# openai/blocksparse

Hardware: NVIDIA H100
Metric: effective TFLOP/s (2*nnz_blocks*bs^2*N, fprop+bprop+updat) (higher is better)
Workload: dtype bf16

## Files before the change

blocksparse_b200/csrc/tc_xprop2.cuh:

```cuda
#pragma once
#include "tc.cuh"

namespace bsmm {

template <int TB, int MI> struct Xp2Shape {
  static constexpr uint32_t XBYTES = MI * 64 * 32 * 2;
  static constexpr uint32_t WBYTES = 32 * 32 * 2;
  static constexpr uint32_t STAGE = (XBYTES + TB * WBYTES + 1023) / 1024 * 1024;
  static constexpr size_t SMEM = XP_STAGES * STAGE + SMEM_ALIGN_SLACK;
};
constexpr int XP2_REC = 8;

struct Xprop2Params {
  const int32_t* tile_off;
  const int32_t* ent;
  int n_out;
  int w_absent;
  void* y;
  long long y_pitch;
  int N;
};

template <int TB, int MI, bool BF16, bool AXIS0, bool BPROP>
__global__ void __launch_bounds__(XP_THREADS)
tc_xprop2_kernel(const Xprop2Params p, const __grid_constant__ XpropTmaps maps) {
  using Sh = Xp2Shape<TB, MI>;
  constexpr int ST = XP_STAGES, NW = TB * 32;
  extern __shared__ uint8_t smem_raw[];
  __shared__ uint64_t full[ST];
  const uint32_t base = aligned_smem_base(smem_raw);
  const int tid = threadIdx.x, warp = tid / 32, lane = tid % 32;
  const int nt = blockIdx.x, t = blockIdx.y;
  const int first = p.tile_off[t], count = p.tile_off[t + 1] - first;
  const int32_t* ent = p.ent + (size_t)first * XP2_REC;

  auto issue = [&](int e) {
    const int32_t* r = ent + e * XP2_REC;
    const uint32_t st = base + (uint32_t)(e % ST) * Sh::STAGE;
    uint64_t* bar = &full[e % ST];
    ptx::mbar_expect_tx(bar, Sh::XBYTES + TB * Sh::WBYTES);
    if (!AXIS0) {
      ptx::tma_load_2d(st, &maps.x, bar, r[0] * 32, nt * MI * 64);
    } else {
#pragma unroll
      for (int m = 0; m < MI; ++m) ptx::tma_load_2d(st + m * 4096, &maps.x, bar, nt * MI * 64 + m * 64, r[0] * 32);
    }
#pragma unroll
    for (int j = 0; j < TB; ++j) {
      const int wb = r[1 + j];
      ptx::tma_load_2d(st + Sh::XBYTES + j * Sh::WBYTES, &maps.w, bar, 0, (wb < 0 ? p.w_absent : wb) * 32);
    }
  };

  if (tid == 0) {
    for (int i = 0; i < ST; ++i) ptx::mbar_init(&full[i], 1);
    ptx::fence_mbar_init();
    ptx::prefetch_tensormap(&maps.x); ptx::prefetch_tensormap(&maps.w);
  }
  __syncthreads();
  if (tid == 0)
    for (int e = 0; e < count && e < ST; ++e) issue(e);

  float acc[MI][NW / 2];
#pragma unroll
  for (int m = 0; m < MI; ++m)
#pragma unroll
    for (int i = 0; i < NW / 2; ++i) acc[m][i] = 0.f;

  for (int e = 0; e < count; ++e) {
    const uint32_t st = base + (uint32_t)(e % ST) * Sh::STAGE;
    if (!ptx::mbar_wait(&full[e % ST], (uint32_t)(e / ST) & 1)) g_tc_error = 41;
    ptx::wg_fence();
#pragma unroll
    for (int ks = 0; ks < 2; ++ks) {
      const uint64_t bdesc = BPROP ? ptx::make_desc(st + Sh::XBYTES + ks * 32, 16, 512, ptx::SWZ_64B)
                                   : ptx::make_desc(st + Sh::XBYTES + ks * 1024, Sh::WBYTES, 512, ptx::SWZ_64B);
#pragma unroll
      for (int m = 0; m < MI; ++m) {
        const uint64_t adesc = AXIS0 ? ptx::make_desc(st + m * 4096 + ks * 2048, 4096, 1024, ptx::SWZ_128B)
                                     : ptx::make_desc(st + m * 64 * 64 + ks * 32, 16, 512, ptx::SWZ_64B);
        ptx::wgmma<BF16, AXIS0 ? 1 : 0, BPROP ? 0 : 1, NW>(acc[m], adesc, bdesc);
      }
    }
    ptx::wg_commit();
    ptx::wg_wait<1>();
    __syncthreads();
    if (tid == 0 && e >= 1 && e - 1 + ST < count) issue(e - 1 + ST);
  }
  ptx::wg_wait<0>();
#pragma unroll
  for (int m = 0; m < MI; ++m) ptx::wg_fence_regs(acc[m]);

  uint16_t* y = reinterpret_cast<uint16_t*>(p.y);
#pragma unroll
  for (int m = 0; m < MI; ++m)
#pragma unroll
    for (int h = 0; h < 2; ++h) {
      const long long n = (long long)nt * MI * 64 + m * 64 + warp * 16 + lane / 4 + 8 * h;
      if (n >= p.N) continue;
#pragma unroll
      for (int j = 0; j < NW / 8; ++j) {
        const int cl = 8 * j + 2 * (lane % 4);
        const int o = t * TB + cl / 32;
        if (o >= p.n_out) continue;
        const int col = o * 32 + cl % 32;
        const float a = acc[m][4 * j + 2 * h], b = acc[m][4 * j + 2 * h + 1];
        if (!AXIS0) {
          *reinterpret_cast<uint32_t*>(y + n * p.y_pitch + col) = pack2<BF16>(a, b);
        } else {
          y[(long long)col * p.y_pitch + n] = pack1<BF16>(a);
          y[(long long)(col + 1) * p.y_pitch + n] = pack1<BF16>(b);
        }
      }
    }
}

template <int TB, int MI, bool BF16, bool AXIS0, bool BPROP>
int launch_tc_xprop2(const Xprop2Params& p, const XpropTmaps& maps, int n_tiles, cudaStream_t s) {
  auto kern = tc_xprop2_kernel<TB, MI, BF16, AXIS0, BPROP>;
  constexpr size_t smem = Xp2Shape<TB, MI>::SMEM;
  static thread_local uint64_t configured = 0;
  if (int e = ensure_dyn_smem(kern, smem, configured)) return e;
  kern<<<dim3((unsigned)((p.N + MI * 64 - 1) / (MI * 64)), (unsigned)n_tiles), XP_THREADS, smem, s>>>(p, maps);
  return check_launch("wgmma_xprop2_bs32");
}

template <int TB, int MI, bool BF16>
int dispatch_tc_xprop2(const Xprop2Params& p, const XpropTmaps& maps, int n_tiles, bool axis0, bool bprop, cudaStream_t s) {
  if (axis0) return bprop ? launch_tc_xprop2<TB, MI, BF16, true, true>(p, maps, n_tiles, s) : launch_tc_xprop2<TB, MI, BF16, true, false>(p, maps, n_tiles, s);
  return bprop ? launch_tc_xprop2<TB, MI, BF16, false, true>(p, maps, n_tiles, s) : launch_tc_xprop2<TB, MI, BF16, false, false>(p, maps, n_tiles, s);
}

inline int tc_xprop2(int dtype, int axis, int bprop, int n_out, int n_in, int blocks, const void* x, const void* w, void* y,
                     int N, const int32_t* sched, int n_tiles, int variant, int ent_off, cudaStream_t s) {
  if (dtype != BSMM_F16 && dtype != BSMM_BF16) return fail(BSMM_E_ARG, "bsmm_xprop: the wide-tile schedule needs a 16-bit dtype");
  if (variant < 1 || variant > 3) return fail(BSMM_E_ARG, "bsmm_xprop: wide-tile variant %d (1..3)", variant);
  const int tb = variant == 3 ? 4 : 2;
  if (sched == nullptr || n_tiles <= 0 || (long long)n_tiles * tb < n_out || ent_off < n_tiles + 3)
    return fail(BSMM_E_ARG, "bsmm_xprop: inconsistent wide-tile schedule (tiles=%d variant=%d entries at %d)", n_tiles, variant, ent_off);
  if (axis == 0 && (N & 7)) { fail(0, "feature_axis 0 needs N %% 8 == 0 for TMA (row pitch multiple of 16 bytes)"); return TC_NOT_APPLICABLE; }
  if (((uintptr_t)x | (uintptr_t)w | (uintptr_t)y) & 15) { fail(0, "pointers must be 16-byte aligned for TMA"); return TC_NOT_APPLICABLE; }
  if (!wgmma_device()) return TC_NOT_APPLICABLE;

  const int rows = variant == 1 ? 64 : 128;
  const uint64_t Cin = (uint64_t)n_in * 32, Cout = (uint64_t)n_out * 32;
  XpropTmaps maps;
  if (axis == 1) {
    if (int e = cached_tmap_2d(&maps.x, dtype, x, Cin, (uint64_t)N, Cin, 32, rows, CU_TENSOR_MAP_SWIZZLE_64B)) return e;
  } else {
    if (int e = cached_tmap_2d(&maps.x, dtype, x, (uint64_t)N, Cin, (uint64_t)N, 64, 32, CU_TENSOR_MAP_SWIZZLE_128B)) return e;
  }
  if (int e = cached_tmap_2d(&maps.w, dtype, w, 32, (uint64_t)blocks * 32, 32, 32, 32, CU_TENSOR_MAP_SWIZZLE_64B)) return e;
  Xprop2Params p;
  p.tile_off = sched + 2; p.ent = sched + ent_off; p.n_out = n_out; p.w_absent = blocks;
  p.y = y; p.y_pitch = axis == 0 ? (long long)N : (long long)Cout; p.N = N;
  const bool bf = dtype == BSMM_BF16, a0 = axis == 0, bp = bprop != 0;
  switch (variant) {
    case 1: return bf ? dispatch_tc_xprop2<2, 1, true>(p, maps, n_tiles, a0, bp, s) : dispatch_tc_xprop2<2, 1, false>(p, maps, n_tiles, a0, bp, s);
    case 2: return bf ? dispatch_tc_xprop2<2, 2, true>(p, maps, n_tiles, a0, bp, s) : dispatch_tc_xprop2<2, 2, false>(p, maps, n_tiles, a0, bp, s);
    default: return bf ? dispatch_tc_xprop2<4, 2, true>(p, maps, n_tiles, a0, bp, s) : dispatch_tc_xprop2<4, 2, false>(p, maps, n_tiles, a0, bp, s);
  }
}

}
```

blocksparse_b200/lut.py:

```python
import numpy as np

SEG_MAX = (1 << 63) - 1


def ceil_div(x, y):
    return -(-x // y)


def z_order_2d(x, y):
    x = np.asarray(x, dtype=np.uint64)
    y = np.asarray(y, dtype=np.uint64)
    code = np.zeros(np.broadcast(x, y).shape, dtype=np.uint64)
    for bit in range(32):
        b = np.uint64(bit)
        code |= ((x >> b) & np.uint64(1)) << np.uint64(2 * bit)
        code |= ((y >> b) & np.uint64(1)) << np.uint64(2 * bit + 1)
    return code if code.shape else int(code)


def _group(outs, n_out):
    counts = np.bincount(outs, minlength=n_out).astype(np.int64)
    starts = np.concatenate(([0], np.cumsum(counts)[:-1]))
    return counts, starts


def row_lut(outs, ins, wids, n_out):
    nnz = len(outs)
    counts, starts = _group(outs, n_out)
    lut = np.empty((n_out + nnz, 2), dtype=np.int32)
    lut[:n_out, 0] = n_out + starts
    lut[:n_out, 1] = counts
    lut[n_out:, 0] = wids
    lut[n_out:, 1] = ins
    return lut, int(counts.max()) if nnz else 0


def segmented_lut(outs, ins, wids, n_out, max_seg, min_seg):
    nnz = len(outs)
    counts, starts = _group(outs, n_out)
    nonempty = np.nonzero(counts)[0]
    empty = np.nonzero(counts == 0)[0]
    n = counts[nonempty]
    if max_seg >= SEG_MAX:
        cuts = np.zeros_like(n)
    else:
        cuts = np.where(n >= min_seg, (n - min_seg) // max_seg, 0)
    segs_per = cuts + 1
    n_seg_ne = int(segs_per.sum())
    grp = np.repeat(np.arange(len(nonempty)), segs_per)
    first_seg = np.concatenate(([0], np.cumsum(segs_per)[:-1]))
    j = np.arange(n_seg_ne) - first_seg[grp]
    is_last = j == cuts[grp]
    seg_len = np.where(is_last, n[grp] - cuts[grp] * max_seg if max_seg < SEG_MAX else n[grp], max_seg).astype(np.int64)
    seg_start = starts[nonempty][grp] + j * (max_seg if max_seg < SEG_MAX else 0)
    split = segs_per > 1
    lock_of_group = np.where(split, np.cumsum(split), 0)
    n_locks = int(split.sum())

    n_seg = n_seg_ne + len(empty)
    lut = np.empty(4 * n_seg + 2 * nnz, dtype=np.int32)
    hdr = lut[:4 * n_seg].reshape(n_seg, 4)
    hdr[:n_seg_ne, 0] = (4 * n_seg) // 2 + seg_start
    hdr[:n_seg_ne, 1] = seg_len
    hdr[:n_seg_ne, 2] = nonempty[grp]
    hdr[:n_seg_ne, 3] = lock_of_group[grp]
    hdr[n_seg_ne:, 0] = (4 * n_seg) // 2 + nnz
    hdr[n_seg_ne:, 1] = 0
    hdr[n_seg_ne:, 2] = empty
    hdr[n_seg_ne:, 3] = 0
    ent = lut[4 * n_seg:].reshape(nnz, 2)
    ent[:, 0] = ins
    ent[:, 1] = wids
    longest = int(seg_len.max()) if n_seg_ne else 0
    return lut, longest * 8, n_seg, n_locks


def lists_from_sorted(outs, ins, wids, n_out):
    counts, starts = _group(outs, n_out)
    ins_l, w_l = ins.tolist(), wids.tolist()
    res, tail = [], []
    for o in range(n_out):
        c, s = int(counts[o]), int(starts[o])
        if c:
            res.append((o, list(zip(ins_l[s:s + c], w_l[s:s + c]))))
        else:
            tail.append((o, []))
    return res + tail


class MatmulLuts(object):

    def __init__(self, layout, z_order=True):
        lay = np.asarray(layout) != 0
        assert lay.ndim == 2
        CB, KB = lay.shape
        self.CB, self.KB = CB, KB
        col_sizes = lay.sum(axis=0)
        if not col_sizes.any():
            raise ValueError("layout has no non-zero blocks")
        big = int(col_sizes.max())
        small = int(col_sizes[col_sizes > 0].min())
        max_seg = max(ceil_div(big, 4), small * 2) if big / small > 2.0 else SEG_MAX
        min_seg = max(ceil_div(max_seg, 4), 4)

        ks, cs = np.nonzero(lay.T)
        cs = cs.astype(np.int64)
        ks = ks.astype(np.int64)
        nnz = len(cs)
        if z_order:
            rank = np.argsort(z_order_2d(cs, ks), kind="stable")
            wid = np.empty(nnz, dtype=np.int64)
            wid[rank] = np.arange(nnz)
            upd_c, upd_k = cs[rank], ks[rank]
        else:
            wid = np.arange(nnz, dtype=np.int64)
            upd_c, upd_k = cs, ks
        self.blocks = nnz
        self.updat_lut = np.stack([upd_c, upd_k], axis=1).astype(np.int32)
        self.updat_list = [tuple(r) for r in self.updat_lut.tolist()]

        by_c = np.argsort(cs, kind="stable")
        f = (ks, cs, wid)
        b = (cs[by_c], ks[by_c], wid[by_c])
        self.fprop_lut, self.fprop_shared, self.fprop_segments, self.fprop_locks = \
            segmented_lut(f[0], f[1], f[2], KB, max_seg, min_seg)
        self.bprop_lut, self.bprop_shared, self.bprop_segments, self.bprop_locks = \
            segmented_lut(b[0], b[1], b[2], CB, max_seg, min_seg)
        self.fprop_list = lists_from_sorted(f[0], f[1], f[2], KB)
        self.bprop_list = lists_from_sorted(b[0], b[1], b[2], CB)
        self.fprop_rows, self.fprop_max = row_lut(f[0], f[1], f[2], KB)
        self.bprop_rows, self.bprop_max = row_lut(b[0], b[1], b[2], CB)
        self._f, self._b = f, b

    def updat_schedule(self, bsize, k_per_tile=None, n_cta=None):
        return build_updat_schedule(self.updat_lut, self.CB, self.KB, bsize, k_per_tile, n_cta)

    def wide_schedule(self, bprop, blocks_per_tile):
        outs, ins, wids = self._b if bprop else self._f
        n_out = self.CB if bprop else self.KB
        return build_wide_schedule(outs, ins, wids, n_out, blocks_per_tile)

    def pair_schedule(self, bprop, blocks_per_tile, w_per_group, n_tiles, n_ntiles, n_ctas, bsize=32):
        outs, ins, wids = self._b if bprop else self._f
        n_out = self.CB if bprop else self.KB
        return build_pair_schedule(outs, ins, wids, n_out, blocks_per_tile, w_per_group, n_tiles, n_ntiles, n_ctas, bsize)

    def pair_tile_schedule(self, bprop, blocks_per_tile, bsize, w_per_group, n_tiles):
        outs, ins, wids = self._b if bprop else self._f
        n_out = self.CB if bprop else self.KB
        return build_pair_tile_schedule(outs, ins, wids, n_out, blocks_per_tile, bsize, w_per_group, n_tiles)

    def tile_schedule(self, bprop, blocks_per_tile, bsize=32, w_per_group=8, n_tiles=None, n_ntiles=None):
        outs, ins, wids = self._b if bprop else self._f
        n_out = self.CB if bprop else self.KB
        return build_tile_schedule(outs, ins, wids, n_out, blocks_per_tile, bsize, w_per_group, n_tiles, n_ntiles)


WIDE_REC = 8


def build_wide_schedule(outs, ins, wids, n_out, blocks_per_tile):
    T = int(blocks_per_tile)
    assert 1 <= T <= WIDE_REC - 1
    outs = np.asarray(outs, dtype=np.int64)
    ins = np.asarray(ins, dtype=np.int64)
    wids = np.asarray(wids, dtype=np.int64)
    n_tiles = max(1, ceil_div(n_out, T))
    n_in = int(ins.max()) + 1 if len(ins) else 1
    key = (outs // T) * n_in + ins
    uniq, inv = np.unique(key, return_inverse=True)
    tile_of = uniq // n_in
    offsets = np.searchsorted(tile_of, np.arange(n_tiles + 1))
    ent_off = ceil_div(3 + n_tiles, WIDE_REC) * WIDE_REC
    sched = np.full(ent_off + WIDE_REC * len(uniq), -1, dtype=np.int32)
    sched[0:2] = (n_tiles, T)
    sched[2:3 + n_tiles] = offsets
    ent = sched[ent_off:].reshape(len(uniq), WIDE_REC)
    ent[:, 0] = uniq % n_in
    ent[inv, 1 + outs % T] = wids
    return sched, n_tiles, ent_off


GROUP_INTS = 32
GROUP_MAX_W = 8
GROUP_MAX_RUNS = 8


def pick_tile_count(n_out, n_ntiles, cta_slots, max_blocks_per_tile):
    lo = ceil_div(n_out, max_blocks_per_tile)
    best = None
    for n_kt in range(lo, min(n_out, 2 * lo) + 1):
        tiles = n_ntiles * n_kt
        waves = ceil_div(tiles, cta_slots)
        cost = waves * (n_out / float(n_kt) + 1.5)
        if best is None or cost < best[0]:
            best = (cost, n_kt)
    return best[1]


def tile_order(tile_cost, n_ntiles):
    cost = np.asarray(tile_cost, dtype=np.float64)
    n_kt = len(cost)
    top = cost.max() if n_kt and cost.max() > 0 else 1.0
    bucket = np.floor(8.0 * cost / top).astype(np.int64)
    kt = np.tile(np.arange(n_kt), n_ntiles)
    nt = np.repeat(np.arange(n_ntiles), n_kt)
    order = np.lexsort((kt, nt, -bucket[kt]))
    return (nt[order] * n_kt + kt[order]).astype(np.int32)


def build_tile_schedule(outs, ins, wids, n_out, blocks_per_tile, bsize=32, w_per_group=8, n_tiles=None, n_ntiles=None):
    T = int(blocks_per_tile)
    assert 1 <= w_per_group <= GROUP_MAX_W
    if n_tiles is None:
        n_tiles = ceil_div(n_out, T)
    n_tiles = int(n_tiles)
    assert n_tiles * T >= n_out
    bounds = (np.arange(n_tiles + 1, dtype=np.int64) * n_out) // n_tiles
    assert int(np.diff(bounds).max()) <= T
    outs = np.asarray(outs, dtype=np.int64)
    ins = np.asarray(ins, dtype=np.int64)
    wids = np.asarray(wids, dtype=np.int64)
    nnz = len(outs)
    tile = np.searchsorted(bounds, outs, side="right") - 1
    order = np.lexsort((outs, ins, tile))
    tile_s, ins_s, outs_s, w_s = tile[order], ins[order], outs[order], wids[order]
    slot_s = outs_s - bounds[tile_s]

    new_cluster = np.ones(nnz, dtype=bool)
    if nnz:
        new_cluster[1:] = (tile_s[1:] != tile_s[:-1]) | (ins_s[1:] != ins_s[:-1])
    cluster_id = np.cumsum(new_cluster) - 1
    cluster_start = np.nonzero(new_cluster)[0]
    pos_in_cluster = np.arange(nnz) - cluster_start[cluster_id]
    new_group = new_cluster | (pos_in_cluster % w_per_group == 0)
    group_id = np.cumsum(new_group) - 1
    g_first = np.nonzero(new_group)[0]
    n_groups = len(g_first)
    g_count = np.diff(np.concatenate((g_first, [nnz])))
    pos_in_group = np.arange(nnz) - g_first[group_id]

    accumulate = np.ones(nnz, dtype=np.int64)

    new_run = np.ones(nnz, dtype=bool)
    if nnz:
        new_run[1:] = new_group[1:] | (slot_s[1:] != slot_s[:-1] + 1)
    run_first = np.nonzero(new_run)[0]
    run_len = np.diff(np.concatenate((run_first, [nnz])))
    run_group = group_id[run_first]
    runs_per_group = np.bincount(run_group, minlength=n_groups)
    run_first_of_group = np.concatenate(([0], np.cumsum(runs_per_group)[:-1]))
    run_pos = np.arange(len(run_first)) - run_first_of_group[run_group]
    assert runs_per_group.max(initial=0) <= GROUP_MAX_RUNS

    groups_per_tile = np.bincount(tile_s[g_first], minlength=n_tiles)
    tile_first_group = np.concatenate(([0], np.cumsum(groups_per_tile)[:-1]))
    touched = np.zeros(n_tiles, dtype=np.int64)
    np.bitwise_or.at(touched, tile, np.int64(1) << (outs - bounds[tile]))

    hdr_ints = 4 + 4 * n_tiles
    grp_off = ceil_div(hdr_ints, GROUP_INTS) * GROUP_INTS
    sched = np.zeros(grp_off + GROUP_INTS * n_groups, dtype=np.int32)
    sched[0:4] = (n_tiles, T, n_groups, nnz)
    th = sched[4:hdr_ints].reshape(n_tiles, 4)
    th[:, 0] = tile_first_group
    th[:, 1] = groups_per_tile
    th[:, 2] = bounds[:-1]
    th[:, 3] = np.diff(bounds) | (touched << 8)
    gr = sched[grp_off:].reshape(n_groups, GROUP_INTS)
    gr[:, 0] = ins_s[g_first]
    gr[:, 1] = g_count | (runs_per_group << 8)
    gr[group_id, 4 + pos_in_group] = w_s
    wbytes16 = (bsize * bsize * 2) >> 4
    r0 = pos_in_group[run_first] * wbytes16 | ((slot_s[run_first] * bsize) << 16)
    r1 = (((run_len * bsize) >> 3) << 17) | accumulate[run_first]
    gr[run_group, 12 + run_pos] = r0
    gr[run_group, 20 + run_pos] = r1
    if n_ntiles is not None:
        w_per_tile = np.bincount(tile, minlength=n_tiles) if nnz else np.zeros(n_tiles, dtype=np.int64)
        cost = 4.0 * groups_per_tile + 1.0 * w_per_tile + 4.0
        order = tile_order(cost, int(n_ntiles))
        order_off = len(sched)
        return np.concatenate((sched, order)), grp_off, order_off
    return sched, grp_off


def build_pair_tile_schedule(outs, ins, wids, n_out, blocks_per_tile, bsize, w_per_group, n_tiles):
    T, WPG = int(blocks_per_tile), int(w_per_group)
    assert 1 <= WPG <= GROUP_MAX_W
    n_tiles = int(n_tiles)
    assert n_tiles * T >= n_out
    bounds = (np.arange(n_tiles + 1, dtype=np.int64) * n_out) // n_tiles
    outs = np.asarray(outs, dtype=np.int64); ins = np.asarray(ins, dtype=np.int64); wids = np.asarray(wids, dtype=np.int64)
    tile = np.searchsorted(bounds, outs, side="right") - 1
    n_even = n_tiles + (n_tiles & 1)
    wbytes16 = (bsize * bsize * 2) >> 4
    max_run = 256 // bsize
    per_tile = [dict() for _ in range(n_even)]
    order = np.lexsort((outs, ins, tile))
    for t, c, o, w in zip(tile[order].tolist(), ins[order].tolist(), outs[order].tolist(), wids[order].tolist()):
        per_tile[t].setdefault(c, []).append((o - int(bounds[t]), w))
    recs = [[] for _ in range(n_even)]

    def records(entries, in_block, n_rec):
        out = []
        for r in range(n_rec):
            chunk = entries[r * WPG:(r + 1) * WPG]
            rec = [0] * GROUP_INTS
            rec[0] = in_block
            runs = []
            for pos, (slot, w) in enumerate(chunk):
                rec[4 + pos] = w
                if runs and runs[-1][1] + runs[-1][2] == slot and runs[-1][2] < max_run:
                    runs[-1][2] += 1
                else:
                    runs.append([pos, slot, 1])
            assert len(runs) <= GROUP_MAX_RUNS
            rec[1] = len(chunk) | (len(runs) << 8)
            for i, (pos, slot, ln) in enumerate(runs):
                rec[12 + i] = (pos * wbytes16) | ((slot * bsize) << 16)
                rec[20 + i] = (((ln * bsize) >> 3) << 17) | 1
            out.append(rec)
        return out

    for P in range(n_even // 2):
        a, b = per_tile[2 * P], per_tile[2 * P + 1]
        for c in sorted(set(a) | set(b)):
            ea, eb = a.get(c, []), b.get(c, [])
            n_rec = max(ceil_div(len(ea), WPG), ceil_div(len(eb), WPG), 1)
            recs[2 * P] += records(ea, c, n_rec)
            recs[2 * P + 1] += records(eb, c, n_rec)
    groups_per_tile = np.array([len(r) for r in recs], dtype=np.int64)
    tile_first_group = np.concatenate(([0], np.cumsum(groups_per_tile)[:-1]))
# ... 301 lines not shown
```

blocksparse_b200/matmul.py:

```python
import ctypes
import os

import numpy as np
import torch

from . import _lib
from .checkers import MatmulCheckers
from .lut import MatmulLuts

_X2_VARIANTS = {1: 2, 2: 2, 3: 4}
_X2_FORCE = int(os.environ.get("BSMM_XPROP2", "0"))
_PAIR_TILES = int(os.environ.get("BSMM_PAIR_TILES", "0"))
_PAD8 = int(os.environ.get("BSMM_PAD8", "1"))


def _as_2d(t, axis, feat):
    if axis == 0:
        if t.shape[0] != feat:
            raise ValueError("expected feature dim %d on axis 0, got shape %s" % (feat, tuple(t.shape)))
        return t.reshape(feat, -1)
    if t.shape[-1] != feat:
        raise ValueError("expected feature dim %d on the last axis, got shape %s" % (feat, tuple(t.shape)))
    return t.reshape(-1, feat)


class BlocksparseMatMul(MatmulCheckers):

    def __getstate__(self):
        return (self.layout, self.bsize, self.axis, self.z_order, self.name)

    def __setstate__(self, state):
        self.__init__(*state)

    def __init__(self, layout, block_size=32, feature_axis=0, z_order=True, name=None):
        if feature_axis not in (0, 1) or block_size not in (8, 16, 32, 64):
            raise ValueError("Unsupported block size with this feature axis")
        layout = np.asarray(layout)
        if layout.ndim != 2:
            raise ValueError("layout must be 2-D")
        self.axis, self.bsize = feature_axis, block_size
        luts = MatmulLuts(layout, z_order=z_order)
        self._luts = luts
        for k in ("updat_list", "updat_lut", "fprop_list", "bprop_list", "fprop_lut", "bprop_lut",
                  "fprop_shared", "bprop_shared", "fprop_segments", "bprop_segments",
                  "fprop_locks", "bprop_locks", "blocks", "CB", "KB"):
            setattr(self, k, getattr(luts, k))
        self.z_order = z_order
        self.name = name or "BlocksparseMatMul"
        self.flops = self.blocks * block_size * block_size * 2
        self.w_shape = (self.blocks, block_size, block_size)
        self.g_shape = (self.blocks,)
        self.count = 0
        self.C, self.K = self.CB * block_size, self.KB * block_size
        self.sparsity = round(float(self.blocks) / float(self.CB * self.KB), 3)
        self.layout = layout != 0
        self._dev = {}
        self._shadow = None
        if block_size == 8 and _PAD8 and self.CB % 2 == 0 and self.KB % 2 == 0:
            big = self.layout.reshape(self.CB // 2, 2, self.KB // 2, 2).any(axis=(1, 3))
            sh = BlocksparseMatMul(big.astype(np.int32), block_size=16, feature_axis=feature_axis, z_order=z_order, name=self.name + "/pad16")
            big_id = -np.ones(big.shape, dtype=np.int64)
            big_id[sh.updat_lut[:, 0], sh.updat_lut[:, 1]] = np.arange(sh.blocks)
            cs, ks = self.updat_lut[:, 0].astype(np.int64), self.updat_lut[:, 1].astype(np.int64)
            inv = big_id[cs // 2, ks // 2] * 4 + (cs % 2) * 2 + (ks % 2)
            sub = -np.ones(sh.blocks * 4, dtype=np.int32)
            sub[inv] = np.arange(self.blocks, dtype=np.int32)
            self._shadow, self._sub_map, self._inv_map = sh, sub, inv.astype(np.int32)

    def i_shape(self, N):
        return (N, self.C) if self.axis else (self.C, N)

    def o_shape(self, N):
        return (N, self.K) if self.axis else (self.K, N)

    def block_coord(self, block):
        return self.updat_list[block]

    def identity_init(self, scale=1.0, dtype=torch.float32, device="cuda"):
        device = torch.device(device)
        if device.type != "cuda":
            raise _lib.BsmmError("identity_init runs on the GPU (no CPU path)")
        if device.index is None:
            device = torch.device("cuda", torch.cuda.current_device())
        W = torch.empty(self.w_shape, dtype=dtype, device=device)
        d = self._device_luts(device)
        with torch.cuda.device(device):
            rc = _lib.load().bsmm_identity_init(_lib.dtype_code(dtype), self.bsize, self.blocks, d["updat"].data_ptr(), self.CB, self.KB,
                                                W.data_ptr(), float(scale), _lib.stream_ptr())
        _lib.check(rc, "bsmm_identity_init")
        return W

    def ortho_init(self, dtype=torch.float32, device="cuda", rng=None):
        rng = rng or np.random
        bs = self.bsize
        W = np.empty(self.w_shape, dtype=np.float32)
        if self.sparsity < 1.0:
            for k, col in self.fprop_list:
                if not col:
                    continue
                shape = (len(col) * bs, bs)
                a = rng.normal(0.0, 1.0, shape).astype(np.float32)
                u, _, v = np.linalg.svd(a, full_matrices=False)
                if u.shape != shape:
                    u = v
                for i, (c, w) in enumerate(col):
                    W[w] = u[i * bs:(i + 1) * bs, :]
        else:
            shape = (self.C, self.K)
            a = rng.normal(0.0, 1.0, shape).astype(np.float32)
            u, _, v = np.linalg.svd(a, full_matrices=False)
            if u.shape != shape:
                u = v
            for w, (c, k) in enumerate(self.updat_list):
                W[w] = u[c * bs:(c + 1) * bs, k * bs:(k + 1) * bs]
        return torch.as_tensor(W).to(dtype).to(device)

    def l2_normalize(self, W, gain=None, epsilon=1e-12, dtype=None):
        return _L2NormalizeFunction.apply(W, gain, self, float(epsilon), dtype or W.dtype)

    def checker_init(self, dtype=torch.float32, device="cuda"):
        cs, ks = self.updat_lut[:, 0], self.updat_lut[:, 1]
        return torch.as_tensor(((cs & 1) ^ (ks & 1) ^ 1).astype(np.float32), device=device).to(dtype)

    def prune(self, param, gate):
        gate_np = gate.detach().cpu().numpy() if torch.is_tensor(gate) else np.asarray(gate)
        keep = gate_np != 0.0
        for w in np.nonzero(~keep)[0]:
            c, k = self.updat_list[w]
            self.layout[c, k] = False
        idx = torch.as_tensor(np.nonzero(keep)[0], device=param.device)
        new_gate = torch.ones(int(keep.sum()), dtype=gate.dtype if torch.is_tensor(gate) else torch.float32,
                              device=param.device)
        return param.index_select(0, idx), new_gate

    def _device_luts(self, device):
        key = (device.type, device.index)
        d = self._dev.get(key)
        if d is None:
            d = {
                "fprop": torch.as_tensor(self._luts.fprop_rows, device=device),
                "bprop": torch.as_tensor(self._luts.bprop_rows, device=device),
                "updat": torch.as_tensor(self.updat_lut, device=device),
            }
            if self.bsize in (16, 32, 64):
                us, uoff = self._luts.updat_schedule(self.bsize, n_cta=_lib.grid_sms(device))
                d["updat_sched"] = torch.as_tensor(us, device=device)
                d["updat_tiles"], d["updat_kt"] = int(us[0]), int(us[2])
            self._dev[key] = d
        return d

    def fprop(self, x, w, gate=None, flags=0):
        return self._xprop(x, w, False, gate, flags)

    def bprop(self, dy, w, gate=None, flags=0):
        return self._xprop(dy, w, True, gate, flags)

    def _pad_maps(self, device):
        d = self._device_luts(device)
        if "sub_map" not in d:
            d["sub_map"] = torch.as_tensor(self._sub_map, device=device)
            d["inv_map"] = torch.as_tensor(self._inv_map, device=device)
        return d["sub_map"], d["inv_map"]

    def _padded_weights(self, w, gate):
        sub, _ = self._pad_maps(w.device)
        sh = self._shadow
        w16 = torch.empty(sh.w_shape, dtype=w.dtype, device=w.device)
        g = None if gate is None else gate.to(torch.float32).contiguous()
        _lib.check(_lib.load().bsmm_pad_blocks(_lib.dtype_code(w.dtype), self.bsize, sh.blocks, sub.data_ptr(), w.contiguous().data_ptr(),
                                               _lib.ptr(g), w16.data_ptr(), _lib.stream_ptr()), "bsmm_pad_blocks")
        return w16

    @_lib.guarded
    def _xprop(self, x, w, bprop, gate, flags):
        lib = _lib.load()
        if not x.is_cuda:
            raise _lib.BsmmError("BlocksparseMatMul needs CUDA tensors (no CPU path)")
        if self._shadow is not None and x.dtype != torch.float32 and not (flags & _lib.FLAG_FORCE_GENERIC):
            if tuple(w.shape) != self.w_shape or w.dtype != x.dtype:
                raise ValueError("w must have shape %s and the dtype of x" % (self.w_shape,))
            return self._shadow._xprop(x, self._padded_weights(w, gate), bprop, None, flags)
        feat_in, feat_out = (self.K, self.C) if bprop else (self.C, self.K)
        x2 = x if (x.dim() == 2 and x.is_contiguous() and x.shape[self.axis] == feat_in) else _as_2d(x, self.axis, feat_in).contiguous()
        if not w.is_contiguous():
            w = w.contiguous()
        if w.shape != self.w_shape:
            raise ValueError("w must have shape %s, got %s" % (self.w_shape, tuple(w.shape)))
        if w.dtype != x.dtype:
            raise ValueError("x and w must have the same dtype")
        N = x2.shape[1] if self.axis == 0 else x2.shape[0]
        d = self._device_luts(x.device)
        lut = d["bprop" if bprop else "fprop"]
        n_in, n_out = (self.KB, self.CB) if bprop else (self.CB, self.KB)
        sched, sched_tiles, tile_arg, sched_off = None, 0, 0, 0
        if self.bsize == 32 and x.dtype != torch.float32:
            if _X2_FORCE in _X2_VARIANTS:
                key = ("wide", bool(bprop), _X2_VARIANTS[_X2_FORCE])
                if key not in d:
                    arr, n_tiles, off = self._luts.wide_schedule(bprop, _X2_VARIANTS[_X2_FORCE])
                    d[key] = (torch.as_tensor(arr, device=x.device), n_tiles, off)
                sched, sched_tiles, sched_off = d[key]
                tile_arg = (1 << 16) | (_X2_FORCE << 8)
            elif _PAIR_TILES:
                tile_arg = 1 << 12
        y2 = torch.empty((feat_out, N) if self.axis == 0 else (N, feat_out), dtype=x.dtype, device=x.device)
        if gate is not None:
            gate = gate.to(torch.float32).contiguous()
            if self.bsize in (16, 32, 64) and x.dtype != torch.float32 and not (flags & _lib.FLAG_FORCE_GENERIC):
                wg = torch.empty_like(w)
                _lib.check(lib.bsmm_gate_weights(_lib.dtype_code(w.dtype), self.bsize, self.blocks, w.data_ptr(),
                                                 gate.data_ptr(), wg.data_ptr(), _lib.stream_ptr()), "bsmm_gate_weights")
                w, gate = wg, None
        rc = lib.bsmm_xprop(_lib.dtype_code(x.dtype), self.axis, self.bsize, int(bprop),
                            lut.data_ptr(), n_out, n_in, self.blocks,
                            x2.data_ptr(), w.data_ptr(), y2.data_ptr(), N,
                            _lib.ptr(gate),
                            _lib.ptr(sched), sched_tiles, tile_arg, sched_off, 0, 0, 0,
                            flags, _lib.stream_ptr())
        _lib.check(rc, "bsmm_xprop")
        if self.axis == 0:
            return y2.reshape((feat_out,) + tuple(x.shape[1:]))
        return y2.reshape(tuple(x.shape[:-1]) + (feat_out,))

    @_lib.guarded
    def updat(self, xs, dys, dw=None, alpha=1.0, gate=None, dw_gated=False, dw_dtype=None, flags=0):
        lib = _lib.load()
        if torch.is_tensor(xs):
            xs, dys = [xs], [dys]
        if len(xs) != len(dys) or not 1 <= len(xs) <= _lib.MAX_PAIRS:
            raise ValueError("need 1..%d (x, dy) pairs" % _lib.MAX_PAIRS)
        x0 = xs[0]
        if not x0.is_cuda:
            raise _lib.BsmmError("BlocksparseMatMul needs CUDA tensors (no CPU path)")
        ax = self.axis
        xs2 = [x if (x.dim() == 2 and x.is_contiguous() and x.shape[ax] == self.C) else _as_2d(x, ax, self.C).contiguous() for x in xs]
        dys2 = [e if (e.dim() == 2 and e.is_contiguous() and e.shape[ax] == self.K) else _as_2d(e, ax, self.K).contiguous() for e in dys]
        N = xs2[0].shape[1] if self.axis == 0 else xs2[0].shape[0]
        for a, b in zip(xs2, dys2):
            if a.dtype != x0.dtype or b.dtype != x0.dtype:
                raise ValueError("all x / dy tensors must share one dtype")
            if (a.shape[1] if self.axis == 0 else a.shape[0]) != N or (b.shape[1] if self.axis == 0 else b.shape[0]) != N:
                raise ValueError("all x / dy tensors must share the minibatch size")
        if self._shadow is not None and x0.dtype != torch.float32 and not (flags & _lib.FLAG_FORCE_GENERIC):
            dw16 = self._shadow.updat(xs, dys, alpha=alpha, dw_dtype=torch.float32, flags=flags)
            _, inv = self._pad_maps(x0.device)
            acc = dw is not None
            if dw is None:
                dw = torch.empty(self.w_shape, dtype=dw_dtype or x0.dtype, device=x0.device)
            elif tuple(dw.shape) != self.w_shape or not dw.is_contiguous():
                raise ValueError("dw must be a contiguous tensor of shape %s" % (self.w_shape,))
            g = gate.to(torch.float32).contiguous() if (gate is not None and dw_gated) else None
            _lib.check(lib.bsmm_unpad_blocks(_lib.F32, _lib.dtype_code(dw.dtype), self.bsize, self.blocks, inv.data_ptr(), dw16.data_ptr(),
                                             _lib.ptr(g), dw.data_ptr(), int(acc), _lib.stream_ptr()), "bsmm_unpad_blocks")
            return dw
        if dw is None:
            out_dtype = dw_dtype or x0.dtype
            dw = torch.empty(self.w_shape, dtype=out_dtype, device=x0.device)
            beta = 0.0
        else:
            if tuple(dw.shape) != self.w_shape or not dw.is_contiguous():
                raise ValueError("dw must be a contiguous tensor of shape %s" % (self.w_shape,))
            beta = 1.0
        if gate is not None:
            gate = gate.to(torch.float32).contiguous()
        xp, ep = _lib.ptr_array(xs2), _lib.ptr_array(dys2)
        d = self._device_luts(x0.device)
        rc = lib.bsmm_updat(_lib.dtype_code(x0.dtype), _lib.dtype_code(dw.dtype), self.axis, self.bsize,
                            d["updat"].data_ptr(), self.blocks, self.CB, self.KB,
                            xp, ep, len(xs2), dw.data_ptr(), N, float(alpha), beta,
                            _lib.ptr(gate), int(bool(dw_gated)),
                            _lib.ptr(d.get("updat_sched")), d.get("updat_tiles", 0), d.get("updat_kt", 0), 0,
                            flags, _lib.stream_ptr())
        _lib.check(rc, "bsmm_updat")
        return dw

    @_lib.guarded
    def gate_grad(self, dw, w):
        lib = _lib.load()
        dg = torch.empty(self.blocks, dtype=torch.float32, device=w.device)
        dw = dw.to(w.dtype).contiguous()
        rc = lib.bsmm_gate_grad(_lib.dtype_code(w.dtype), self.bsize, self.blocks, dw.data_ptr(),
                                w.contiguous().data_ptr(), dg.data_ptr(), _lib.stream_ptr())
        _lib.check(rc, "bsmm_gate_grad")
        return dg

    def matmul(self, I, W, gate=None, gate_grad=False, dw_gated=False, name=None, bench=0):
        return self.__call__(I, W, gate=gate, gate_grad=gate_grad, dw_gated=dw_gated, name=name, bench=bench)

    def __call__(self, I, W, gate=None, gate_grad=False, dw_gated=False, name=None, bench=0):
        self.count += 1
        if bench:
            self._bench_op("fprop", lambda: self.fprop(I, W, gate), I, bench, name or self.name)
        return _BsmmFunction.apply(I, W, gate, self, bool(gate_grad), bool(dw_gated), int(bench), name or self.name)

    def _bench_op(self, what, fn, I, repeat, name):
        lib = _lib.load()
        timer = ctypes.c_void_p()
        _lib.check(lib.bsmm_timer_create(ctypes.byref(timer)), "timer_create")
        fn()
        _lib.check(lib.bsmm_timer_begin(timer, _lib.stream_ptr()), "timer_begin")
        for _ in range(repeat):
            fn()
        ms = ctypes.c_float()
        _lib.check(lib.bsmm_timer_end(timer, _lib.stream_ptr(), ctypes.byref(ms)), "timer_end")
        lib.bsmm_timer_destroy(timer)
        N = I.numel() // (self.K if what == "bprop" else self.C)
        ms_per = ms.value / repeat
        gflops = self.flops * N / (ms_per * 1e6)
        print("%s %s ms: %.4f gflops: %.0f" % (name, what, ms_per, gflops))
        return ms_per


class _BsmmFunction(torch.autograd.Function):

    @staticmethod
    def forward(ctx, x, w, gate, bsmm, gate_grad, dw_gated, bench=0, name=None):
        ctx.bsmm, ctx.gate_grad, ctx.dw_gated, ctx.bench, ctx.name = bsmm, gate_grad, dw_gated, bench, name
        ctx.save_for_backward(x, w, gate)
        return bsmm.fprop(x, w, gate)

    @staticmethod
    def backward(ctx, dy):
        x, w, gate = ctx.saved_tensors
        bsmm = ctx.bsmm
        dy = dy.contiguous()
        if ctx.bench:
            bsmm._bench_op("bprop", lambda: bsmm.bprop(dy, w, gate), dy, ctx.bench, ctx.name)
            bsmm._bench_op("updat", lambda: bsmm.updat([x], [dy], gate=gate, dw_gated=ctx.dw_gated), x, ctx.bench, ctx.name)
        dx = bsmm.bprop(dy, w, gate) if ctx.needs_input_grad[0] else None
        dw = dg = None
        want_dg = gate is not None and ctx.gate_grad and ctx.needs_input_grad[2]
        if want_dg:
            raw = bsmm.updat([x], [dy])
            dg = bsmm.gate_grad(raw, w).to(gate.dtype)
            dw = raw * gate.to(raw.dtype).view(-1, 1, 1)
        elif ctx.needs_input_grad[1]:
            pending = _pending_group(bsmm, w)
            if pending is not None:
                dw = pending.add(x, dy, gate, ctx.dw_gated)
            else:
                dw = bsmm.updat([x], [dy], gate=gate, dw_gated=ctx.dw_gated)
        return dx, dw, dg, None, None, None, None, None



_groups = {}


class _Pending(object):
    def __init__(self, bsmm, w, group_size):
        self.bsmm, self.w, self.group_size = bsmm, w, group_size
        self.xs, self.dys = [], []
        self.gate, self.dw_gated = None, False
        self.dw = None
        self.launches = 0

    def add(self, x, dy, gate, dw_gated):
# ... 234 lines not shown
```

Baseline: 174.6.

## Add grouped wide-tile xprop kernel that skips absent weight blocks, auto-selected

Adds a grouped xprop kernel. Each CTA covers 128 rows and a group of 4 output blocks, staging each input block once and loading only the weight blocks that are present, using a per-entry mask kept in a shared-memory LUT. A host heuristic estimates staged bytes against the narrow path and CTA count per SM, and picks the grouped kernel by default when it should reduce traffic. It also widens the schedule record to 16 ints and adds per-chunk LUT staging with syncs. The costs are extra pipeline drains at LUT chunk boundaries and possibly less parallelism.

Result: faster. 202.6 (median of 6 runs) (+16.0%).

```diff
diff --git a/blocksparse_b200/csrc/tc_xprop2.cuh b/blocksparse_b200/csrc/tc_xprop2.cuh
--- a/blocksparse_b200/csrc/tc_xprop2.cuh
+++ b/blocksparse_b200/csrc/tc_xprop2.cuh
@@ -9,7 +9,7 @@
   static constexpr uint32_t STAGE = (XBYTES + TB * WBYTES + 1023) / 1024 * 1024;
   static constexpr size_t SMEM = XP_STAGES * STAGE + SMEM_ALIGN_SLACK;
 };
-constexpr int XP2_REC = 8;
+constexpr int XP2_REC = 16;
 
 struct Xprop2Params {
   const int32_t* tile_off;
@@ -131,11 +131,164 @@
   return bprop ? launch_tc_xprop2<TB, MI, BF16, false, true>(p, maps, n_tiles, s) : launch_tc_xprop2<TB, MI, BF16, false, false>(p, maps, n_tiles, s);
 }
 
+template <int G> struct XpgShape {
+  static constexpr uint32_t XBYTES = 128 * 32 * 2;
+  static constexpr uint32_t WBYTES = 32 * 32 * 2;
+  static constexpr uint32_t STAGE = XBYTES + G * WBYTES;
+  static constexpr size_t SMEM = XP_STAGES * STAGE + SMEM_ALIGN_SLACK;
+};
+
+constexpr int XPG_LUT = 128;
+
+template <int G, bool BF16, bool AXIS0, bool BPROP>
+__global__ void __launch_bounds__(XP_THREADS)
+tc_xprop_grouped_kernel(const Xprop2Params p, const __grid_constant__ XpropTmaps maps, const int n_tiles) {
+  using Sh = XpgShape<G>;
+  constexpr int ST = XP_STAGES;
+  extern __shared__ uint8_t smem_raw[];
+  __shared__ uint64_t full[ST];
+  const uint32_t base = aligned_smem_base(smem_raw);
+  const int tid = threadIdx.x, warp = tid / 32, lane = tid % 32;
+  const int nt = blockIdx.x / n_tiles, t = blockIdx.x % n_tiles;
+  const int first = p.tile_off[t], count = p.tile_off[t + 1] - first;
+  const int32_t* ent = p.ent + (size_t)first * XP2_REC;
+  __shared__ int32_t rec[XPG_LUT][G + 2];
+
+  auto issue = [&](int c0, int e) {
+    const int32_t* r = rec[e];
+    const int g = c0 + e;
+    const uint32_t st = base + (uint32_t)(g % ST) * Sh::STAGE;
+    uint64_t* bar = &full[g % ST];
+    const uint32_t mask = (uint32_t)r[G + 1];
+    ptx::mbar_expect_tx(bar, Sh::XBYTES + (uint32_t)__popc(mask) * Sh::WBYTES);
+    const int c = r[0];
+    if (!AXIS0) {
+      ptx::tma_load_2d(st, &maps.x, bar, c * 32, nt * 128);
+    } else {
+      ptx::tma_load_2d(st, &maps.x, bar, nt * 128, c * 32);
+      ptx::tma_load_2d(st + Sh::XBYTES / 2, &maps.x, bar, nt * 128 + 64, c * 32);
+    }
+#pragma unroll
+    for (int j = 0; j < G; ++j)
+      if (mask >> j & 1) ptx::tma_load_2d(st + Sh::XBYTES + j * Sh::WBYTES, &maps.w, bar, 0, r[1 + j] * 32);
+  };
+
+  if (tid == 0) {
+    for (int i = 0; i < ST; ++i) ptx::mbar_init(&full[i], 1);
+    ptx::fence_mbar_init();
+    ptx::prefetch_tensormap(&maps.x); ptx::prefetch_tensormap(&maps.w);
+  }
+
+  float acc[2][G][16];
+#pragma unroll
+  for (int m = 0; m < 2; ++m)
+#pragma unroll
+    for (int j = 0; j < G; ++j)
+#pragma unroll
+      for (int i = 0; i < 16; ++i) acc[m][j][i] = 0.f;
+
+  for (int c0 = 0; c0 < count; c0 += XPG_LUT) {
+    const int n = min(count - c0, XPG_LUT);
+    __syncthreads();
+    for (int i = tid; i < n; i += XP_THREADS) {
+      const int32_t* r = ent + (size_t)(c0 + i) * XP2_REC;
+      int32_t mask = 0;
+      rec[i][0] = __ldg(r);
+#pragma unroll
+      for (int j = 0; j < G; ++j) {
+        const int32_t wb = __ldg(r + 1 + j);
+        rec[i][1 + j] = wb;
+        mask |= (int32_t)(wb >= 0) << j;
+      }
+      rec[i][G + 1] = mask;
+    }
+    __syncthreads();
+    if (tid == 0)
+      for (int e = 0; e < n && e < ST; ++e) issue(c0, e);
+    for (int e = 0; e < n; ++e) {
+      const int g = c0 + e;
+      const uint32_t st = base + (uint32_t)(g % ST) * Sh::STAGE;
+      const uint32_t mask = (uint32_t)rec[e][G + 1];
+      if (!ptx::mbar_wait(&full[g % ST], (uint32_t)(g / ST) & 1)) g_tc_error = 45;
+      ptx::wg_fence();
+#pragma unroll
+      for (int j = 0; j < G; ++j) {
+        if (mask >> j & 1) {
+#pragma unroll
+          for (int ks = 0; ks < 2; ++ks) {
+            const uint32_t wb = st + Sh::XBYTES + j * Sh::WBYTES;
+            const uint64_t bdesc = BPROP ? ptx::make_desc(wb + ks * 32, 16, 512, ptx::SWZ_64B)
+                                         : ptx::make_desc(wb + ks * 1024, Sh::WBYTES, 512, ptx::SWZ_64B);
+#pragma unroll
+            for (int m = 0; m < 2; ++m) {
+              const uint64_t adesc = AXIS0 ? ptx::make_desc(st + m * (Sh::XBYTES / 2) + ks * 2048, Sh::XBYTES / 2, 1024, ptx::SWZ_128B)
+                                           : ptx::make_desc(st + m * 64 * 64 + ks * 32, 16, 512, ptx::SWZ_64B);
+              ptx::wgmma<BF16, AXIS0 ? 1 : 0, BPROP ? 0 : 1, 32>(acc[m][j], adesc, bdesc);
+            }
+          }
+        }
+      }
+      ptx::wg_commit();
+      ptx::wg_wait<1>();
+      __syncthreads();
+      if (tid == 0 && e >= 1 && e - 1 + ST < n) issue(c0, e - 1 + ST);
+    }
+    ptx::wg_wait<0>();
+  }
+#pragma unroll
+  for (int m = 0; m < 2; ++m)
+#pragma unroll
+    for (int j = 0; j < G; ++j) ptx::wg_fence_regs(acc[m][j]);
+
+  uint16_t* y = reinterpret_cast<uint16_t*>(p.y);
+#pragma unroll
+  for (int m = 0; m < 2; ++m)
+#pragma unroll
+    for (int h = 0; h < 2; ++h) {
+      const long long n = (long long)nt * 128 + m * 64 + warp * 16 + lane / 4 + 8 * h;
+      if (n >= p.N) continue;
+#pragma unroll
+      for (int j = 0; j < G; ++j) {
+        const int o = t * G + j;
+        if (o >= p.n_out) continue;
+#pragma unroll
+        for (int q = 0; q < 4; ++q) {
+          const int col = o * 32 + 8 * q + 2 * (lane % 4);
+          const float a = acc[m][j][4 * q + 2 * h], b = acc[m][j][4 * q + 2 * h + 1];
+          if (!AXIS0) {
+            *reinterpret_cast<uint32_t*>(y + n * p.y_pitch + col) = pack2<BF16>(a, b);
+          } else {
+            y[(long long)col * p.y_pitch + n] = pack1<BF16>(a);
+            y[(long long)(col + 1) * p.y_pitch + n] = pack1<BF16>(b);
+          }
+        }
+      }
+    }
+}
+
+template <int G, bool BF16, bool AXIS0, bool BPROP>
+int launch_tc_xprop_grouped(const Xprop2Params& p, const XpropTmaps& maps, int n_tiles, cudaStream_t s) {
+  auto kern = tc_xprop_grouped_kernel<G, BF16, AXIS0, BPROP>;
+  constexpr size_t smem = XpgShape<G>::SMEM;
+  static thread_local uint64_t configured = 0;
+  if (int e = ensure_dyn_smem(kern, smem, configured)) return e;
+  const long long ctas = (long long)((p.N + 127) / 128) * n_tiles;
+  if (ctas > 0x7fffffffLL) return fail(BSMM_E_LIMIT, "bsmm_xprop: %lld CTAs exceed the grid limit", ctas);
+  kern<<<dim3((unsigned)ctas), XP_THREADS, smem, s>>>(p, maps, n_tiles);
+  return check_launch("wgmma_xprop_bs32");
+}
+
+template <int G, bool BF16>
+int dispatch_tc_xprop_grouped(const Xprop2Params& p, const XpropTmaps& maps, int n_tiles, bool axis0, bool bprop, cudaStream_t s) {
+  if (axis0) return bprop ? launch_tc_xprop_grouped<G, BF16, true, true>(p, maps, n_tiles, s) : launch_tc_xprop_grouped<G, BF16, true, false>(p, maps, n_tiles, s);
+  return bprop ? launch_tc_xprop_grouped<G, BF16, false, true>(p, maps, n_tiles, s) : launch_tc_xprop_grouped<G, BF16, false, false>(p, maps, n_tiles, s);
+}
+
 inline int tc_xprop2(int dtype, int axis, int bprop, int n_out, int n_in, int blocks, const void* x, const void* w, void* y,
                      int N, const int32_t* sched, int n_tiles, int variant, int ent_off, cudaStream_t s) {
   if (dtype != BSMM_F16 && dtype != BSMM_BF16) return fail(BSMM_E_ARG, "bsmm_xprop: the wide-tile schedule needs a 16-bit dtype");
-  if (variant < 1 || variant > 3) return fail(BSMM_E_ARG, "bsmm_xprop: wide-tile variant %d (1..3)", variant);
-  const int tb = variant == 3 ? 4 : 2;
+  if (variant < 1 || variant > 4) return fail(BSMM_E_ARG, "bsmm_xprop: wide-tile variant %d (1..4)", variant);
+  const int tb = variant >= 3 ? 4 : 2;
   if (sched == nullptr || n_tiles <= 0 || (long long)n_tiles * tb < n_out || ent_off < n_tiles + 3)
     return fail(BSMM_E_ARG, "bsmm_xprop: inconsistent wide-tile schedule (tiles=%d variant=%d entries at %d)", n_tiles, variant, ent_off);
   if (axis == 0 && (N & 7)) { fail(0, "feature_axis 0 needs N %% 8 == 0 for TMA (row pitch multiple of 16 bytes)"); return TC_NOT_APPLICABLE; }
@@ -158,8 +311,9 @@
   switch (variant) {
     case 1: return bf ? dispatch_tc_xprop2<2, 1, true>(p, maps, n_tiles, a0, bp, s) : dispatch_tc_xprop2<2, 1, false>(p, maps, n_tiles, a0, bp, s);
     case 2: return bf ? dispatch_tc_xprop2<2, 2, true>(p, maps, n_tiles, a0, bp, s) : dispatch_tc_xprop2<2, 2, false>(p, maps, n_tiles, a0, bp, s);
-    default: return bf ? dispatch_tc_xprop2<4, 2, true>(p, maps, n_tiles, a0, bp, s) : dispatch_tc_xprop2<4, 2, false>(p, maps, n_tiles, a0, bp, s);
-  }
-}
-
-}
+    case 3: return bf ? dispatch_tc_xprop2<4, 2, true>(p, maps, n_tiles, a0, bp, s) : dispatch_tc_xprop2<4, 2, false>(p, maps, n_tiles, a0, bp, s);
+    default: return bf ? dispatch_tc_xprop_grouped<4, true>(p, maps, n_tiles, a0, bp, s) : dispatch_tc_xprop_grouped<4, false>(p, maps, n_tiles, a0, bp, s);
+  }
+}
+
+}
diff --git a/blocksparse_b200/lut.py b/blocksparse_b200/lut.py
--- a/blocksparse_b200/lut.py
+++ b/blocksparse_b200/lut.py
@@ -156,12 +156,12 @@
         return build_tile_schedule(outs, ins, wids, n_out, blocks_per_tile, bsize, w_per_group, n_tiles, n_ntiles)
 
 
-WIDE_REC = 8
+WIDE_REC = 16
 
 
 def build_wide_schedule(outs, ins, wids, n_out, blocks_per_tile):
     T = int(blocks_per_tile)
-    assert 1 <= T <= WIDE_REC - 1
+    assert 1 <= T <= 8
     outs = np.asarray(outs, dtype=np.int64)
     ins = np.asarray(ins, dtype=np.int64)
     wids = np.asarray(wids, dtype=np.int64)
@@ -179,6 +179,24 @@
     ent[:, 0] = uniq % n_in
     ent[inv, 1 + outs % T] = wids
     return sched, n_tiles, ent_off
+
+
+XPROP_GROUP = 4
+XPROP_GROUP_MAX_BYTES = 0.95
+XPROP_GROUP_MIN_CTAS_PER_SM = 6.0
+
+
+def xprop_staged_bytes(nnz, merged_entries, N):
+    n_tiles = ceil_div(N, 128)
+    return nnz * 10240 * n_tiles, (merged_entries * 8192 + nnz * 2048) * n_tiles
+
+
+def pick_xprop_tile(nnz, merged_entries, n_out, N, n_sm, group=XPROP_GROUP):
+    narrow, grouped = xprop_staged_bytes(nnz, merged_entries, N)
+    ctas = ceil_div(N, 128) * ceil_div(n_out, group)
+    if grouped <= XPROP_GROUP_MAX_BYTES * narrow and ctas >= XPROP_GROUP_MIN_CTAS_PER_SM * n_sm:
+        return group
+    return 1
 
 
 GROUP_INTS = 32
diff --git a/blocksparse_b200/matmul.py b/blocksparse_b200/matmul.py
--- a/blocksparse_b200/matmul.py
+++ b/blocksparse_b200/matmul.py
@@ -6,11 +6,13 @@
 
 from . import _lib
 from .checkers import MatmulCheckers
-from .lut import MatmulLuts
+from .lut import MatmulLuts, WIDE_REC, XPROP_GROUP, pick_xprop_tile
 
 _X2_VARIANTS = {1: 2, 2: 2, 3: 4}
 _X2_FORCE = int(os.environ.get("BSMM_XPROP2", "0"))
 _PAIR_TILES = int(os.environ.get("BSMM_PAIR_TILES", "0"))
+_GROUPED_VARIANTS = {4: 4}
+_XPROP_TILE = None
 _PAD8 = int(os.environ.get("BSMM_PAD8", "1"))
 
 
@@ -149,6 +151,23 @@
             self._dev[key] = d
         return d
 
+    def _wide_schedule(self, d, device, bprop, blocks_per_tile):
+        key = ("wide", bool(bprop), blocks_per_tile)
+        if key not in d:
+            arr, n_tiles, off = self._luts.wide_schedule(bprop, blocks_per_tile)
+            d[key] = (torch.as_tensor(arr, device=device), n_tiles, off, (len(arr) - off) // WIDE_REC)
+        return d[key]
+
+    def xprop_tile(self, bprop, N, device):
+        if _XPROP_TILE is not None:
+            return _XPROP_TILE
+        d = self._device_luts(device)
+        key = ("tile", bool(bprop), N)
+        if key not in d:
+            entries = self._wide_schedule(d, device, bprop, XPROP_GROUP)[3]
+            d[key] = pick_xprop_tile(self.blocks, entries, self.CB if bprop else self.KB, N, _lib.grid_sms(device))
+        return d[key]
+
     def fprop(self, x, w, gate=None, flags=0):
         return self._xprop(x, w, False, gate, flags)
 
@@ -195,14 +214,15 @@
         sched, sched_tiles, tile_arg, sched_off = None, 0, 0, 0
         if self.bsize == 32 and x.dtype != torch.float32:
             if _X2_FORCE in _X2_VARIANTS:
-                key = ("wide", bool(bprop), _X2_VARIANTS[_X2_FORCE])
-                if key not in d:
-                    arr, n_tiles, off = self._luts.wide_schedule(bprop, _X2_VARIANTS[_X2_FORCE])
-                    d[key] = (torch.as_tensor(arr, device=x.device), n_tiles, off)
-                sched, sched_tiles, sched_off = d[key]
+                sched, sched_tiles, sched_off, _ = self._wide_schedule(d, x.device, bprop, _X2_VARIANTS[_X2_FORCE])
                 tile_arg = (1 << 16) | (_X2_FORCE << 8)
             elif _PAIR_TILES:
                 tile_arg = 1 << 12
+            else:
+                tile = self.xprop_tile(bprop, N, x.device)
+                if tile > 1:
+                    sched, sched_tiles, sched_off, _ = self._wide_schedule(d, x.device, bprop, tile)
+                    tile_arg = (1 << 16) | (_GROUPED_VARIANTS[tile] << 8)
         y2 = torch.empty((feat_out, N) if self.axis == 0 else (N, feat_out), dtype=x.dtype, device=x.device)
         if gate is not None:
             gate = gate.to(torch.float32).contiguous()
```
